# kawshik8/GAN-Image-Captioning

Measured on AMD Instinct MI355X. Metric: captions/sec (G+D train step), higher is better.
Workload: dtype bf16; 1 GPU; cfg2: adversarial G+D step, batch 64/GPU, 224x224 images, caption len 20, V=10000, E=H=512, 1-layer LSTM G, CNN-seq D (R=64,F=900), ResNet-50-shaped encoder, --conditional-gan 1; global_batch=64, caption_len=20, image_size=224, vocab=10000, conditional_gan=1, encoder=resnet50, step_impl=fused, parallelism=dp1

## Files before the change

### gan-image-captioning_amd/csrc/gemm.hip

```cpp
#include "gemm.h"
#include "conv3x3.h"
#include "conv1x1_stream.h"
#include "conv1x1_panel.h"
#include "conv1x1_pix.h"
#include "conv_stem.h"
#include "bn_fold.h"
#include "kernels.h"

#include <stdlib.h>

namespace gic {

namespace {

typedef __attribute__((address_space(3))) bf16x4 lds_bf16x4;
typedef unsigned int u32x4 __attribute__((ext_vector_type(4)));
typedef const __attribute__((address_space(1))) u32x4* gptr_u4;

__device__ __attribute__((aligned(16))) unsigned int g_zero16[4] = {0u, 0u, 0u, 0u};
typedef __attribute__((address_space(3))) void* lds_void_ptr;
typedef const __attribute__((address_space(1))) void* gbl_void_ptr;

#ifdef GIC_STAMPS
}
__device__ unsigned long long g_stamp[32];
namespace {
#define STAMP(i) do { if (tid == 0 && blockIdx.y == 0 && (blockIdx.x == 0 || blockIdx.x == gridDim.x - 1)) { \
  const int o_ = blockIdx.x == 0 ? 0 : 16; g_stamp[o_ + 2 * (i)] = __builtin_amdgcn_s_memtime(); g_stamp[o_ + 2 * (i) + 1] = __builtin_amdgcn_s_memrealtime(); } } while (0)
#define DBG d.dbg
#else
#define STAMP(i) do {} while (0)
#define DBG 0
#endif

template <typename T> struct GlobalPtr { typedef const __attribute__((address_space(1))) T* type; };

template <typename TI, typename TO, bool AKC, bool BKC, int BM, int BN, bool VEC, int EPI, bool CONV, bool PIPE>
__global__ __launch_bounds__(256) void gemm_kernel(const GemmDesc d, const int k_tiles_per_split) {
  static_assert(!CONV || (AKC && BKC && VEC), "the implicit-GEMM convolution loader is k-contiguous and vectorised");
  static_assert(!PIPE || (AKC && BKC && VEC), "the LDS-DMA pipeline needs k-contiguous 16-byte chunks");
  constexpr int SZ = sizeof(TI);
  constexpr int BK = 128 / SZ;
  constexpr int VE = 16 / SZ;
  constexpr int SA = PIPE ? 128 : (AKC ? 144 : BM * SZ + 16);
  constexpr int SB = PIPE ? 128 : (BKC ? 144 : BN * SZ + 16);
  constexpr int NSTAGE = PIPE ? 3 : 2;
  constexpr int A_BYTES = AKC ? BM * SA : BK * SA;
  constexpr int B_BYTES = BKC ? BN * SB : BK * SB;
  constexpr int BUF_BYTES = A_BYTES + B_BYTES;
  constexpr int TM = BM / 32, TN = BN / 32;
  constexpr int CA = BM / 32, CB = BN / 32;
  constexpr bool IS_BF16 = (SZ == 2);
  typedef typename GlobalPtr<TI>::type gptr_t;

  constexpr int EPI_BYTES = BM * (BN * (int)sizeof(TO) + 16) + 4 * (BN / 2) * 2 * 4;
  constexpr int SMEM_BYTES = NSTAGE * BUF_BYTES > EPI_BYTES ? NSTAGE * BUF_BYTES : EPI_BYTES;
  __shared__ __attribute__((aligned(16))) unsigned char smem[SMEM_BYTES];

  const int tid = threadIdx.x, lane = tid & 63, w = tid >> 6;
  STAMP(0);
  const int wr = w >> 1, wc = w & 1;
  const int lr = lane & 15, lg = lane >> 4;

  const int tiles_m = (d.M + BM - 1) / BM;
  const int nwg = gridDim.x;
  int bid = blockIdx.x;
  {
    const int q = nwg >> 3, r = nwg & 7, x = bid & 7;
    bid = (x < r ? x * (q + 1) : r * (q + 1) + (x - r) * q) + (bid >> 3);
  }
  const int bm0 = (bid % tiles_m) * BM;
  const int bn0 = (bid / tiles_m) * BN;

  gptr_t A = (gptr_t)d.A;
  gptr_t B = (gptr_t)d.B;
  const int M = d.M, N = d.N, K = d.K;
  const long lda = d.lda, ldb = d.ldb;

  f32x4 acc[TM][TN];
#pragma unroll
  for (int i = 0; i < TM; ++i)
#pragma unroll
    for (int j = 0; j < TN; ++j) acc[i][j] = (f32x4){0.f, 0.f, 0.f, 0.f};

  u32x4 ra[CA], rb[CB];

  long cv_base[CONV ? CA : 1];
  int cv_hi0[CONV ? CA : 1], cv_wi0[CONV ? CA : 1];
  int cv_r = 0, cv_s = 0, cv_c = 0;
  if constexpr (CONV) {
#pragma unroll
    for (int i = 0; i < CA; ++i) {
      const int m = bm0 + ((tid + i * 256) >> 3);
      const int mm = m < M ? m : 0;
      const int wo = mm % d.cWo, t = mm / d.cWo;
      const int ho = t % d.cHo, n = t / d.cHo;
      cv_hi0[i] = m < M ? ho * d.cStride - d.cPad : -(1 << 28);
      cv_wi0[i] = wo * d.cStride - d.cPad;
      cv_base[i] = ((long)n * d.cH + cv_hi0[i]) * d.cW + cv_wi0[i];
    }
    const int kchunk = PIPE ? ((tid & 7) ^ ((tid >> 4) & 7)) : (tid & 7);
    const int k = blockIdx.y * k_tiles_per_split * BK + kchunk * VE;
    cv_c = k % d.cCin;
    const int t = k / d.cCin;
    cv_s = t % d.cKW;
    cv_r = t / d.cKW;
  }

  auto gload = [&](int kt) {
    if constexpr (VEC) {
      const int k0 = kt * BK;
#pragma unroll
      for (int i = 0; i < CA; ++i) {
        const int c = tid + i * 256;
        ra[i] = (u32x4){0u, 0u, 0u, 0u};
        if constexpr (CONV) {
          const int hi = cv_hi0[i] + cv_r, wi = cv_wi0[i] + cv_s;
          if (cv_r < d.cKH && hi >= 0 && hi < d.cH && wi >= 0 && wi < d.cW)
            ra[i] = *(gptr_u4)(A + (cv_base[i] + (long)cv_r * d.cW + cv_s) * d.cCin + cv_c);
        } else if constexpr (AKC) {
          const int m = bm0 + (c >> 3), k = k0 + (c & 7) * VE;
          if (m < M && k < K) ra[i] = *(gptr_u4)(A + (long)m * lda + k);
        } else {
          constexpr int CPR = BM / VE;
          const int k = k0 + c / CPR, m = bm0 + (c % CPR) * VE;
          if (k < K && m < M) ra[i] = *(gptr_u4)(A + (long)k * lda + m);
        }
      }
#pragma unroll
      for (int i = 0; i < CB; ++i) {
        const int c = tid + i * 256;
        rb[i] = (u32x4){0u, 0u, 0u, 0u};
        if constexpr (BKC) {
          const int n = bn0 + (c >> 3), k = k0 + (c & 7) * VE;
          if (n < N && k < K) rb[i] = *(gptr_u4)(B + (long)n * ldb + k);
        } else {
          constexpr int CPR = BN / VE;
          const int k = k0 + c / CPR, n = bn0 + (c % CPR) * VE;
          if (k < K && n < N) rb[i] = *(gptr_u4)(B + (long)k * ldb + n);
        }
      }
      if constexpr (CONV) {
        cv_c += BK;
        while (cv_c >= d.cCin) {
          cv_c -= d.cCin;
          if (++cv_s == d.cKW) { cv_s = 0; ++cv_r; }
        }
      }
    }
  };

  auto sstore = [&](int kt, int buf) {
    unsigned char* sA = smem + buf * BUF_BYTES;
    unsigned char* sB = sA + A_BYTES;
    if constexpr (VEC) {
#pragma unroll
      for (int i = 0; i < CA; ++i) {
        const int c = tid + i * 256;
        if constexpr (AKC) {
          *(u32x4*)(sA + (c >> 3) * SA + (c & 7) * 16) = ra[i];
        } else {
          constexpr int CPR = BM / VE;
          *(u32x4*)(sA + (c / CPR) * SA + (c % CPR) * 16) = ra[i];
        }
      }
#pragma unroll
      for (int i = 0; i < CB; ++i) {
        const int c = tid + i * 256;
        if constexpr (BKC) {
          *(u32x4*)(sB + (c >> 3) * SB + (c & 7) * 16) = rb[i];
        } else {
          constexpr int CPR = BN / VE;
          *(u32x4*)(sB + (c / CPR) * SB + (c % CPR) * 16) = rb[i];
        }
      }
    } else {
      const int k0 = kt * BK;
      for (int e = tid; e < BM * BK; e += 256) {
        TI v = (TI)0.f;
        if constexpr (AKC) {
          const int row = e / BK, kk = e % BK;
          const int m = bm0 + row, k = k0 + kk;
          if (m < M && k < K) v = A[(long)m * lda + k];
          *(TI*)(sA + row * SA + kk * SZ) = v;
        } else {
          const int kk = e / BM, row = e % BM;
          const int m = bm0 + row, k = k0 + kk;
          if (m < M && k < K) v = A[(long)k * lda + m];
          *(TI*)(sA + kk * SA + row * SZ) = v;
        }
      }
      for (int e = tid; e < BN * BK; e += 256) {
        TI v = (TI)0.f;
        if constexpr (BKC) {
          const int row = e / BK, kk = e % BK;
          const int n = bn0 + row, k = k0 + kk;
          if (n < N && k < K) v = B[(long)n * ldb + k];
          *(TI*)(sB + row * SB + kk * SZ) = v;
        } else {
          const int kk = e / BN, row = e % BN;
          const int n = bn0 + row, k = k0 + kk;
          if (n < N && k < K) v = B[(long)k * ldb + n];
          *(TI*)(sB + kk * SB + row * SZ) = v;
        }
      }
    }
  };

  auto issue = [&](int kt, int buf) {
    if constexpr (PIPE) {
      unsigned char* sA = smem + buf * BUF_BYTES;
      unsigned char* sB = sA + A_BYTES;
      const int k0 = kt * BK;
      const int kc = ((tid & 7) ^ ((tid >> 4) & 7)) * VE;
      const int wbase = (tid & ~63) * 16;
#pragma unroll
      for (int i = 0; i < CA; ++i) {
        const int c = tid + i * 256;
        const TI* src = (const TI*)g_zero16;
        if constexpr (CONV) {
          const int hi = cv_hi0[i] + cv_r, wi = cv_wi0[i] + cv_s;
          if (cv_r < d.cKH && hi >= 0 && hi < d.cH && wi >= 0 && wi < d.cW)
            src = (const TI*)d.A + (cv_base[i] + (long)cv_r * d.cW + cv_s) * d.cCin + cv_c;
        } else {
          const int m = bm0 + (c >> 3), k = k0 + kc;
          if (m < M && k < K) src = (const TI*)d.A + (long)m * lda + k;
        }
        __builtin_amdgcn_global_load_lds((gbl_void_ptr)src, (lds_void_ptr)(sA + i * 4096 + wbase), 16, 0, 0);
      }
#pragma unroll
      for (int i = 0; i < CB; ++i) {
        const int c = tid + i * 256;
        const TI* src = (const TI*)g_zero16;
        const int n = bn0 + (c >> 3), k = k0 + kc;
        if (n < N && k < K) src = (const TI*)d.B + (long)n * ldb + k;
        __builtin_amdgcn_global_load_lds((gbl_void_ptr)src, (lds_void_ptr)(sB + i * 4096 + wbase), 16, 0, 0);
      }
      if constexpr (CONV) {
        cv_c += BK;
        while (cv_c >= d.cCin) {
          cv_c -= d.cCin;
          if (++cv_s == d.cKW) { cv_s = 0; ++cv_r; }
        }
      }
    }
  };

  auto compute = [&](int buf) {
    const unsigned char* sA = smem + buf * BUF_BYTES;
    const unsigned char* sB = sA + A_BYTES;
    if constexpr (IS_BF16) {
#pragma unroll
      for (int ks = 0; ks < BK / 32; ++ks) {
        bf16x8 fa[TM], fb[TN];
#pragma unroll
        for (int t = 0; t < TM; ++t) {
          const int r0 = wr * (BM / 2) + t * 16;
          if constexpr (PIPE) {
            fa[t] = *(const bf16x8*)(sA + (r0 + lr) * 128 + (((ks * 4 + lg) ^ (((r0 + lr) >> 1) & 7)) << 4));
          } else if constexpr (AKC) {
            fa[t] = *(const bf16x8*)(sA + (r0 + lr) * SA + ks * 64 + lg * 16);
          } else {
            const unsigned char* p0 = sA + (ks * 32 + lg * 8 + (lr >> 2)) * SA + (r0 + 4 * (lr & 3)) * 2;
            bf16x4 t0 = __builtin_amdgcn_ds_read_tr16_b64_v4bf16((lds_bf16x4*)p0);
            bf16x4 t1 = __builtin_amdgcn_ds_read_tr16_b64_v4bf16((lds_bf16x4*)(p0 + 4 * SA));
            fa[t] = __builtin_shufflevector(t0, t1, 0, 1, 2, 3, 4, 5, 6, 7);
          }
        }
#pragma unroll
        for (int t = 0; t < TN; ++t) {
          const int r0 = wc * (BN / 2) + t * 16;
          if constexpr (PIPE) {
            fb[t] = *(const bf16x8*)(sB + (r0 + lr) * 128 + (((ks * 4 + lg) ^ (((r0 + lr) >> 1) & 7)) << 4));
          } else if constexpr (BKC) {
            fb[t] = *(const bf16x8*)(sB + (r0 + lr) * SB + ks * 64 + lg * 16);
          } else {
            const unsigned char* p0 = sB + (ks * 32 + lg * 8 + (lr >> 2)) * SB + (r0 + 4 * (lr & 3)) * 2;
            bf16x4 t0 = __builtin_amdgcn_ds_read_tr16_b64_v4bf16((lds_bf16x4*)p0);
            bf16x4 t1 = __builtin_amdgcn_ds_read_tr16_b64_v4bf16((lds_bf16x4*)(p0 + 4 * SB));
            fb[t] = __builtin_shufflevector(t0, t1, 0, 1, 2, 3, 4, 5, 6, 7);
          }
        }
#pragma unroll
        for (int i = 0; i < TM; ++i)
#pragma unroll
          for (int j = 0; j < TN; ++j)
            acc[i][j] = __builtin_amdgcn_mfma_f32_16x16x32_bf16(fa[i], fb[j], acc[i][j], 0, 0, 0);
      }
    } else {
      float fa[TM][8], fb[TN][8];
#pragma unroll
      for (int t = 0; t < TM; ++t) {
        const int r0 = wr * (BM / 2) + t * 16;
        if constexpr (AKC) {
          const int sw = PIPE ? (((r0 + lr) >> 1) & 7) : 0;
          const float4 v0 = *(const float4*)(sA + (r0 + lr) * SA + (((2 * lg) ^ sw) << 4));
          const float4 v1 = *(const float4*)(sA + (r0 + lr) * SA + (((2 * lg + 1) ^ sw) << 4));
          fa[t][0] = v0.x; fa[t][1] = v0.y; fa[t][2] = v0.z; fa[t][3] = v0.w;
          fa[t][4] = v1.x; fa[t][5] = v1.y; fa[t][6] = v1.z; fa[t][7] = v1.w;
        } else {
#pragma unroll
          for (int s = 0; s < 8; ++s) fa[t][s] = *(const float*)(sA + (lg * 8 + s) * SA + (r0 + lr) * 4);
        }
      }
#pragma unroll
      for (int t = 0; t < TN; ++t) {
        const int r0 = wc * (BN / 2) + t * 16;
        if constexpr (BKC) {
          const int sw = PIPE ? (((r0 + lr) >> 1) & 7) : 0;
// ... 526 lines not shown
      __syncthreads();
      constexpr int CG = BN / 8;
      const int pc = tid % CG, pr = tid / CG;
      const int n0 = bn0 + pc * 8, m0 = bm0 + pr * 4;
      if (pr < BM / 4 && n0 < N && m0 < M) {
        float keep[4][8];
#pragma unroll
        for (int e = 0; e < 8; ++e) {
          keep[0][e] = keep[1][e] = keep[2][e] = keep[3][e] = 1.f;
          if (!d.mask && d.use_philox && n0 + e < N) {
            uint32_t r0, r1, r2, r3;
            Philox::gen4(d.seed_dev ? *d.seed_dev : d.seed, d.stream, (uint64_t)(m0 >> 2) * (uint64_t)N + (uint64_t)(n0 + e), r0, r1, r2, r3);
            keep[0][e] = Philox::u01(r0) >= d.drop_p ? 1.f : 0.f;
            keep[1][e] = Philox::u01(r1) >= d.drop_p ? 1.f : 0.f;
            keep[2][e] = Philox::u01(r2) >= d.drop_p ? 1.f : 0.f;
            keep[3][e] = Philox::u01(r3) >= d.drop_p ? 1.f : 0.f;
          }
        }
#pragma unroll
        for (int r = 0; r < 4; ++r) {
          const int m = m0 + r;
          if (m >= M) break;
          const float4 h0 = *(const float4*)(sH + (pr * 4 + r) * SH + pc * 8), h1 = *(const float4*)(sH + (pr * 4 + r) * SH + pc * 8 + 4);
          const float h[8] = {h0.x, h0.y, h0.z, h0.w, h1.x, h1.y, h1.z, h1.w};
          const bf16x8 xv = *(const bf16x8*)((const bf16_t*)d.X + (long)m * d.ldx + n0);
          bf16x8 yv;
          unsigned long long kb = 0ull;
#pragma unroll
          for (int e = 0; e < 8; ++e) {
            const bool live = n0 + e < N;
            const float sg = 1.f / (1.f + expf(-h[e]));
            const float y = sg * fmaxf(h[e], 0.f) + (1.f - sg) * (float)xv[e];
            float k = keep[r][e];
            if (d.mask && live) k = (float)d.mask[(long)m * d.ldmask + n0 + e];
            kb |= (unsigned long long)(live ? (unsigned)k : 0u) << (8 * e);
            yv[e] = (bf16_t)(live ? y * k * d.keep_scale : 0.f);
          }
          if (d.Hpre) {
            *(float4*)(d.Hpre + (long)m * d.ldh + n0) = h0;
            *(float4*)(d.Hpre + (long)m * d.ldh + n0 + 4) = h1;
          }
          if (d.mask_out) *(unsigned long long*)(d.mask_out + (long)m * d.ldmask_out + n0) = kb;
          *(bf16x8*)((bf16_t*)C + (long)m * d.ldc + n0) = yv;
        }
      }
      STAMP(5);
      return;
    }
#pragma unroll
    for (int i = 0; i < TM; ++i) {
#pragma unroll
      for (int j = 0; j < TN; ++j) {
        const int n = bn0 + wc * (BN / 2) + j * 16 + lr;
        if (n >= N) continue;
        const float bias = d.bias ? d.bias[n] : 0.f;
        const int mb = bm0 + wr * 32 + i * 16 + lg * 4;
        float keep4[4] = {1.f, 1.f, 1.f, 1.f};
        if (!d.mask && d.use_philox) {
          uint32_t r0, r1, r2, r3;
          Philox::gen4(d.seed_dev ? *d.seed_dev : d.seed, d.stream, (uint64_t)(mb >> 2) * (uint64_t)N + (uint64_t)n, r0, r1, r2, r3);
          keep4[0] = Philox::u01(r0) >= d.drop_p ? 1.f : 0.f;
          keep4[1] = Philox::u01(r1) >= d.drop_p ? 1.f : 0.f;
          keep4[2] = Philox::u01(r2) >= d.drop_p ? 1.f : 0.f;
          keep4[3] = Philox::u01(r3) >= d.drop_p ? 1.f : 0.f;
        }
#pragma unroll
        for (int r = 0; r < 4; ++r) {
          const int m = mb + r;
          if (m >= M) continue;
          const float v = d.alpha * acc[i][j][r] + bias;
          const float x = to_f32<bf16_t>(((const bf16_t*)d.X)[(long)m * d.ldx + n]);
          const float sg = 1.f / (1.f + expf(-v));
          const float y = sg * fmaxf(v, 0.f) + (1.f - sg) * x;
          if (d.Hpre) d.Hpre[(long)m * d.ldh + n] = v;
          float keep = keep4[r];
          if (d.mask) keep = (float)d.mask[(long)m * d.ldmask + n];
          if (d.mask_out) d.mask_out[(long)m * d.ldmask_out + n] = (uint8_t)keep;
          C[(long)m * d.ldc + n] = from_f32<TO>(y * keep * d.keep_scale);
        }
      }
    }
    STAMP(5);
    return;
  }
  unsigned char* sC = smem;
  float* sStat = (float*)(smem + BM * SC);
#pragma unroll
  for (int j = 0; j < TN; ++j) {
    const int nl = wc * (BN / 2) + j * 16 + lr;
    const int n = bn0 + nl;
    const float bias = (d.bias && n < N) ? d.bias[n] : 0.f;
    float st_s = 0.f, st_q = 0.f;
#pragma unroll
    for (int i = 0; i < TM; ++i) {
#pragma unroll
      for (int r = 0; r < 4; ++r) {
        const int ml = wr * 32 + i * 16 + lg * 4 + r;
        const float v = d.alpha * acc[i][j][r] + bias;
        *(TO*)(sC + ml * SC + nl * OSZ) = from_f32<TO>(v);
        if (EPI == EPI_BNSTATS && bm0 + ml < M) { st_s += v; st_q += v * v; }
      }
    }
    if constexpr (EPI == EPI_BNSTATS) {
      st_s += __shfl_xor(st_s, 16, 64); st_q += __shfl_xor(st_q, 16, 64);
      st_s += __shfl_xor(st_s, 32, 64); st_q += __shfl_xor(st_q, 32, 64);
      if (lg == 0) { sStat[(w * (BN / 2) + j * 16 + lr) * 2] = st_s; sStat[(w * (BN / 2) + j * 16 + lr) * 2 + 1] = st_q; }
    }
  }
  __syncthreads();
  STAMP(4);
  if constexpr (EPI == EPI_BNSTATS) {
    if (tid < BN) {
      const int cwc = tid / (BN / 2), cl = tid % (BN / 2), n = bn0 + tid;
      if (n < N) {
        float s0 = 0.f, q0 = 0.f;
#pragma unroll
        for (int r = 0; r < 4; ++r) {
          s0 += sStat[((r * 2 + cwc) * (BN / 2) + cl) * 2];
          q0 += sStat[((r * 2 + cwc) * (BN / 2) + cl) * 2 + 1];
        }
        float* stp = d.stats + (long)(blockIdx.x % d.stats_nrep) * 2 * N;
        atomicAdd(&stp[n], s0);
        atomicAdd(&stp[N + n], q0);
      }
    }
  }
  constexpr int CPR = BN / OVE;
  for (int c = tid; c < BM * CPR; c += NT) {
    const int ml = c / CPR, cc = c % CPR;
    const int m = bm0 + ml, n = bn0 + cc * OVE;
    if (m < M && n < N) {
      u32x4 v = *(const u32x4*)(sC + ml * SC + cc * 16);
      if (d.accumulate) {
        const u32x4 o = *(const u32x4*)(C + (long)m * d.ldc + n);
        TO* pv = (TO*)&v;
        const TO* po = (const TO*)&o;
#pragma unroll
        for (int e = 0; e < OVE; ++e) pv[e] = from_f32<TO>(to_f32<TO>(pv[e]) + to_f32<TO>(po[e]));
      }
      *(u32x4*)(C + (long)m * d.ldc + n) = v;
    }
  }
  STAMP(5);
}

template <typename TO, int EPI, bool CONV>
bool try_tile8(const GemmDesc& d_in, hipStream_t stream) {
  static const bool off = getenv("GIC_NO_TILE8") != nullptr;
  GemmDesc d = d_in;
  constexpr int OVE = 16 / (int)sizeof(TO);
  if (off || d.M < 128) return false;
  if (EPI != EPI_HIGHWAY && ((d.N % OVE) || (d.ldc % OVE) || (((uintptr_t)d.C) & 15))) return false;
  if (EPI == EPI_HIGHWAY && d.in_dtype != DT_BF16) return false;
  if (!CONV && ((long)cdiv(d.M, 128) * cdiv(d.N, 64) < 128 || d.K < 256)) return false;
  const long a_elems = CONV ? (long)(d.M / (d.cHo * d.cWo)) * d.cH * d.cW * d.cCin : (long)(d.M - 1) * d.lda + d.K;
  const long b_elems = (long)(d.N - 1) * d.ldb + d.K;
  if (a_elems * 2 >= (1l << 31) || b_elems * 2 >= (1l << 31)) return false;
  const long big_tiles = (long)cdiv(d.M, 128) * cdiv(d.N, 128);
  static const int big_min = [] { const char* e = getenv("GIC_TILE8_BIG_MIN"); return e ? atoi(e) : 160; }();
  static const int ns2_tiles = [] { const char* e = getenv("GIC_TILE8_NS2_TILES"); return e ? atoi(e) : 256; }();
  static const int min_nk = [] { const char* e = getenv("GIC_TILE8_MIN_NK"); return e ? atoi(e) : 1; }();
  if (cdiv(d.K, 64) < min_nk) return false;
  const unsigned ab = (unsigned)(a_elems * 2), bb = (unsigned)(b_elems * 2);
  d.n_fast = xcd_share_a(2 * (a_elems < (long)d.M * d.K ? a_elems : (long)d.M * d.K), 2l * d.N * d.K, cdiv(d.N, d.N >= 128 ? 128 : 64));
  if constexpr (EPI == EPI_BNSTATS && CONV) {
    if (d.in_stats && d.res) {
      if (d.cKH != 1 || d.cKW != 1 || d.cStride != 1 || d.cPad != 0 || d.cCin % 8 || d.cCin > 2048 || !d.in_gamma || !d.in_beta ||
          d.in_inv_count <= 0.f || (d.res_stats && (!d.res_gamma || !d.res_beta || d.res_inv_count <= 0.f)))
        return false;
      const bool n128 = d.N >= 128;
      const long tiles = n128 ? big_tiles : (long)cdiv(d.M, 128) * cdiv(d.N, 64);
      const dim3 grid((unsigned)tiles), block(512);
      static const int res_ns = [] { const char* e = getenv("GIC_TILE8_RES_NS"); return e ? atoi(e) : 1; }();
      if (d.cCin <= 512) {
        if (res_ns == 1) {
          if (n128) hipLaunchKernelGGL((tile8_kernel<TO, 128, EPI, CONV, 1, true, true, 512>), grid, block, 0, stream, d, ab, bb);
          else hipLaunchKernelGGL((tile8_kernel<TO, 64, EPI, CONV, 1, true, true, 512>), grid, block, 0, stream, d, ab, bb);
        } else {
          if (n128) hipLaunchKernelGGL((tile8_kernel<TO, 128, EPI, CONV, 2, true, true, 512>), grid, block, 0, stream, d, ab, bb);
          else hipLaunchKernelGGL((tile8_kernel<TO, 64, EPI, CONV, 2, true, true, 512>), grid, block, 0, stream, d, ab, bb);
        }
      } else {
        if (res_ns == 1) {
          if (n128) hipLaunchKernelGGL((tile8_kernel<TO, 128, EPI, CONV, 1, true, true, 2048>), grid, block, 0, stream, d, ab, bb);
          else hipLaunchKernelGGL((tile8_kernel<TO, 64, EPI, CONV, 1, true, true, 2048>), grid, block, 0, stream, d, ab, bb);
        } else {
          if (n128) hipLaunchKernelGGL((tile8_kernel<TO, 128, EPI, CONV, 2, true, true, 2048>), grid, block, 0, stream, d, ab, bb);
          else hipLaunchKernelGGL((tile8_kernel<TO, 64, EPI, CONV, 2, true, true, 2048>), grid, block, 0, stream, d, ab, bb);
        }
      }
      return true;
    }
    if (d.in_stats) {
      if (d.cCin % 8 || d.cCin > 1024 || !d.in_gamma || !d.in_beta || d.in_inv_count <= 0.f) return false;
      const int nk = cdiv(d.K, 64);
      const bool n128 = d.N >= 128 && big_tiles >= big_min;
      const long tiles = n128 ? big_tiles : (long)cdiv(d.M, 128) * cdiv(d.N, 64);
      const dim3 grid((unsigned)tiles), block(512);
      if (nk <= 4 && tiles > 512) {
        if (n128) hipLaunchKernelGGL((tile8_kernel<TO, 128, EPI, CONV, 1, true>), grid, block, 0, stream, d, ab, bb);
        else hipLaunchKernelGGL((tile8_kernel<TO, 64, EPI, CONV, 1, true>), grid, block, 0, stream, d, ab, bb);
      } else if (tiles > 256) {
        if (n128) hipLaunchKernelGGL((tile8_kernel<TO, 128, EPI, CONV, 2, true>), grid, block, 0, stream, d, ab, bb);
        else hipLaunchKernelGGL((tile8_kernel<TO, 64, EPI, CONV, 2, true>), grid, block, 0, stream, d, ab, bb);
      } else {
        if (n128) hipLaunchKernelGGL((tile8_kernel<TO, 128, EPI, CONV, 4, true>), grid, block, 0, stream, d, ab, bb);
        else hipLaunchKernelGGL((tile8_kernel<TO, 64, EPI, CONV, 4, true>), grid, block, 0, stream, d, ab, bb);
      }
      return true;
    }
  }
  static const int ns1_nk = [] { const char* e = getenv("GIC_TILE8_NS1_NK"); return e ? atoi(e) : 4; }();
  const int nk8 = cdiv(d.K, 64);
  if (EPI != EPI_HIGHWAY && nk8 <= ns1_nk && (d.N >= 128 ? big_tiles : (long)cdiv(d.M, 128) * cdiv(d.N, 64)) > 512) {
    if (d.N >= 128) hipLaunchKernelGGL((tile8_kernel<TO, 128, EPI, CONV, 1>), dim3((unsigned)big_tiles), dim3(512), 0, stream, d, ab, bb);
    else hipLaunchKernelGGL((tile8_kernel<TO, 64, EPI, CONV, 1>), dim3((unsigned)(cdiv(d.M, 128) * cdiv(d.N, 64))), dim3(512), 0, stream, d, ab, bb);
    return true;
  }
  if (d.N >= 128 && big_tiles >= big_min) {
    if (big_tiles > ns2_tiles) hipLaunchKernelGGL((tile8_kernel<TO, 128, EPI, CONV, 2>), dim3((unsigned)big_tiles), dim3(512), 0, stream, d, ab, bb);
    else hipLaunchKernelGGL((tile8_kernel<TO, 128, EPI, CONV, 4>), dim3((unsigned)big_tiles), dim3(512), 0, stream, d, ab, bb);
  } else {
    const long tiles = (long)cdiv(d.M, 128) * cdiv(d.N, 64);
    if (tiles > ns2_tiles) hipLaunchKernelGGL((tile8_kernel<TO, 64, EPI, CONV, 2>), dim3((unsigned)tiles), dim3(512), 0, stream, d, ab, bb);
    else hipLaunchKernelGGL((tile8_kernel<TO, 64, EPI, CONV, 4>), dim3((unsigned)tiles), dim3(512), 0, stream, d, ab, bb);
  }
  return true;
}


__global__ void zero2d_kernel(float* __restrict__ C, long ldc, int M, int N) {
  const long total = (long)M * N;
  for (long i = (long)blockIdx.x * blockDim.x + threadIdx.x; i < total; i += (long)gridDim.x * blockDim.x)
    C[(i / N) * ldc + (i % N)] = 0.f;
}

template <typename TI, typename TO, bool AKC, bool BKC, int BM, int BN, bool VEC, int EPI, bool CONV = false>
int launch(const GemmDesc& d, hipStream_t stream) {
  constexpr int BK = 128 / (int)sizeof(TI);
  const int tiles = cdiv(d.M, BM) * cdiv(d.N, BN);
  const int nk = cdiv(d.K, BK);
  int splits = 1;
  if (EPI == EPI_PLAIN && sizeof(TI) == 2 && sizeof(TO) == 4 && !d.no_split) {
    if (tiles < 24 && nk >= 8) {
      splits = 256 / tiles;
      if (splits > nk / 2) splits = nk / 2;
      if (splits > 16) splits = 16;
    } else if (tiles <= 192 && nk >= 32) {
      splits = 512 / tiles;
      if (splits > nk / 8) splits = nk / 8;
      if (splits > 16) splits = 16;
    } else if (!AKC && !BKC && tiles <= 192 && nk >= 16) {
      splits = 512 / tiles;
      if (splits > nk / 4) splits = nk / 4;
    } else if (tiles <= 320 && nk >= 64) {
      splits = 768 / tiles;
    }
    if (splits < 1) splits = 1;
    if (det_mode()) splits = (d.accumulate || splits < 2) ? 1 : 2;
  }
  int per = cdiv(nk, splits);
  splits = cdiv(nk, per);
  if (splits > 1 && !d.accumulate && !d.c_zeroed) {
    const long total = (long)d.M * d.N;
    const int g = (int)((total + 255) / 256 > 1024 ? 1024 : (total + 255) / 256);
    hipLaunchKernelGGL(zero2d_kernel, dim3(g), dim3(256), 0, stream, (float*)d.C, d.ldc, d.M, d.N);
  }
  constexpr bool CAN_PIPE = AKC && BKC && VEC;
  static const bool no_pipe = getenv("GIC_GEMM_NO_PIPE") != nullptr;
  const bool pipe = CAN_PIPE && per >= 6 && (long)tiles * splits <= 2 * 256 + 8 && !no_pipe;
  if constexpr (CAN_PIPE) {
    if (pipe) {
      hipLaunchKernelGGL((gemm_kernel<TI, TO, AKC, BKC, BM, BN, VEC, EPI, CONV, true>), dim3(tiles, splits), dim3(256), 0, stream, d, per);
      GIC_CHECK_LAUNCH("gemm");
      return GIC_OK;
    }
  }
  hipLaunchKernelGGL((gemm_kernel<TI, TO, AKC, BKC, BM, BN, VEC, EPI, CONV, false>), dim3(tiles, splits), dim3(256), 0, stream, d, per);
  GIC_CHECK_LAUNCH("gemm");
  return GIC_OK;
}

int big_tile_min() {
  static const int v = [] { const char* e = getenv("GIC_GEMM_BIG_MIN"); return e ? atoi(e) : 192; }();
  return v;
}

template <typename TI, typename TO, bool AKC, bool BKC, int EPI>
int pick_tile(const GemmDesc& d, bool vec, hipStream_t stream) {
  const long big_tiles = (long)cdiv(d.M, 128) * cdiv(d.N, 128);
  const bool big = big_tiles >= big_tile_min() && d.M >= 128 && d.N >= 128;
  if (big) {
    return vec ? launch<TI, TO, AKC, BKC, 128, 128, true, EPI>(d, stream)
               : launch<TI, TO, AKC, BKC, 128, 128, false, EPI>(d, stream);
  }
  return vec ? launch<TI, TO, AKC, BKC, 64, 64, true, EPI>(d, stream)
             : launch<TI, TO, AKC, BKC, 64, 64, false, EPI>(d, stream);
}

template <typename TI, typename TO, int EPI>
int pick_layout(const GemmDesc& d, bool vec, hipStream_t stream) {
  if constexpr (sizeof(TI) == 2) {
    if (d.a_kc && d.b_kc && vec && try_tile8<TO, EPI, false>(d, stream)) { GIC_CHECK_LAUNCH("gemm tile8"); return GIC_OK; }
  }
  if (d.a_kc && d.b_kc) return pick_tile<TI, TO, true, true, EPI>(d, vec, stream);
  if constexpr (EPI == EPI_PLAIN) {
    if (d.a_kc && !d.b_kc) return pick_tile<TI, TO, true, false, EPI>(d, vec, stream);
    if (!d.a_kc && !d.b_kc) return pick_tile<TI, TO, false, false, EPI>(d, vec, stream);
  }
  set_last_error("gemm: unsupported layout a_kc=%d b_kc=%d epi=%d", d.a_kc, d.b_kc, d.epi);
  return GIC_ERR_UNSUPPORTED;
}

template <typename TI, typename TO, int EPI>
int pick_conv(const GemmDesc& d, hipStream_t stream) {
  if constexpr (sizeof(TI) == 2 && sizeof(TO) == 2 && EPI == EPI_BNSTATS) {
    if (try_conv_stem(d, stream)) { GIC_CHECK_LAUNCH("conv stem"); return GIC_OK; }
    if (try_conv3x3_patch(d, stream)) { GIC_CHECK_LAUNCH("conv3x3 patch"); return GIC_OK; }
    if (try_conv1x1_stream(d, stream)) { GIC_CHECK_LAUNCH("conv1x1 stream"); return GIC_OK; }
    if (d.stats_only) return GIC_ERR_UNSUPPORTED;
    if (try_conv1x1_pix(d, stream)) { GIC_CHECK_LAUNCH("conv1x1 pix"); return GIC_OK; }
    if (try_conv1x1_panel(d, stream)) { GIC_CHECK_LAUNCH("conv1x1 panel"); return GIC_OK; }
    if (d.in_stats && d.cKH * d.cKW > 1) return GIC_ERR_UNSUPPORTED;
  }
  if constexpr (sizeof(TI) == 2) {
    if (try_tile8<TO, EPI, true>(d, stream)) { GIC_CHECK_LAUNCH("conv tile8"); return GIC_OK; }
  }
  if (d.in_stats) return GIC_ERR_UNSUPPORTED;
  const long big_tiles = (long)cdiv(d.M, 128) * cdiv(d.N, 128);
  if (big_tiles >= big_tile_min() && d.N >= 128) return launch<TI, TO, true, true, 128, 128, true, EPI, true>(d, stream);
  return launch<TI, TO, true, true, 64, 64, true, EPI, true>(d, stream);
}

template <typename TI, typename TO>
int pick_epi(const GemmDesc& d, bool vec, hipStream_t stream) {
  if (d.conv) {
    if (!vec || !d.a_kc || !d.b_kc) { set_last_error("gemm: convolution needs 16-B aligned NHWC / KRSC operands"); return GIC_ERR_UNSUPPORTED; }
    if constexpr (sizeof(TI) == sizeof(TO)) {
      if (d.epi == EPI_BNSTATS) return pick_conv<TI, TO, EPI_BNSTATS>(d, stream);
      if (d.epi == EPI_PLAIN) return pick_conv<TI, TO, EPI_PLAIN>(d, stream);
    }
    set_last_error("gemm: unsupported convolution epilogue / dtype");
    return GIC_ERR_UNSUPPORTED;
  }
  if (d.epi == EPI_PLAIN) return pick_layout<TI, TO, EPI_PLAIN>(d, vec, stream);
  if (d.epi == EPI_HIGHWAY) return pick_layout<TI, TO, EPI_HIGHWAY>(d, vec, stream);
  set_last_error("gemm: unknown epilogue %d", d.epi);
  return GIC_ERR_UNSUPPORTED;
}

bool aligned16(const void* p) { return (((uintptr_t)p) & 15) == 0; }

}

int gemm_gumbelmax(const GemmDesc& d0, hipStream_t stream) {
  GemmDesc d = d0;
  static const bool off = getenv("GIC_NO_TILE8") != nullptr || getenv("GIC_NO_FUSED_GUMBELMAX") != nullptr;
  GIC_CHECK_ARG(d.A && d.B && d.gm_rowkey && d.gm_bias, "gemm_gumbelmax: null operand");
  if (off || d.in_dtype != DT_BF16 || !d.a_kc || !d.b_kc || d.M < 128 || d.M % 4 || d.K % 8 || d.lda % 8 || d.ldb % 8 || !aligned16(d.A) ||
      !aligned16(d.B) || !aligned16(d.gm_bias) || (d.gm_u && (!aligned16(d.gm_u) || d.gm_ldu % 4)) || !(d.gm_temperature > 0.f))
    return GIC_ERR_UNSUPPORTED;
  const long a_elems = (long)(d.M - 1) * d.lda + d.K, b_elems = (long)(d.N - 1) * d.ldb + d.K;
  const long tiles = (long)cdiv(d.M, 128) * cdiv(d.N, 128);
  if (a_elems * 2 >= (1l << 31) || b_elems * 2 >= (1l << 31) || d.N < 128 || tiles < 160) return GIC_ERR_UNSUPPORTED;
  d.epi = EPI_GUMBELMAX;
  d.n_fast = xcd_share_a(2l * d.M * d.K, 2l * d.N * d.K, cdiv(d.N, 128));
  const unsigned ab = (unsigned)(a_elems * 2), bb = (unsigned)(b_elems * 2);
  if (tiles > 256) hipLaunchKernelGGL((tile8_kernel<float, 128, EPI_GUMBELMAX, false, 2>), dim3((unsigned)tiles), dim3(512), 0, stream, d, ab, bb);
  else hipLaunchKernelGGL((tile8_kernel<float, 128, EPI_GUMBELMAX, false, 4>), dim3((unsigned)tiles), dim3(512), 0, stream, d, ab, bb);
  GIC_CHECK_LAUNCH("gemm gumbelmax");
  return GIC_OK;
}

int gemm(const GemmDesc& d0, hipStream_t stream) {
  GemmDesc d = d0;
#ifdef GIC_STAMPS
  { const char* e = getenv("GIC_GEMM_DBG"); if (e) d.dbg = atoi(e); }
#endif
  GIC_CHECK_ARG(d.A && d.B && d.C, "gemm: null operand");
  GIC_CHECK_ARG(d.M >= 0 && d.N >= 0 && d.K >= 0, "gemm: negative dim");
  if (d.M == 0 || d.N == 0) return GIC_OK;
  {
    static const bool log = getenv("GIC_GEMM_LOG") != nullptr;
    if (log && !d.conv)
      fprintf(stderr, "[gemm] M=%d N=%d K=%d a_kc=%d b_kc=%d in=%d out=%d epi=%d acc=%d\n", d.M, d.N, d.K, d.a_kc, d.b_kc, d.in_dtype, d.out_dtype, d.epi,
              d.accumulate);
  }
  if (d.epi == EPI_HIGHWAY) GIC_CHECK_ARG(d.X, "gemm: highway epilogue needs X");
  const int sz = dtype_size(d.in_dtype);
  const int ve = 16 / sz;
  bool vec = aligned16(d.A) && aligned16(d.B) && (d.lda % ve == 0) && (d.ldb % ve == 0);
  if (d.conv) {
    const bool chunk_ok = (d.cCin % ve == 0) || (d.cPad == 0 && ve % d.cCin == 0 && (d.cKW * d.cCin) % ve == 0);
    GIC_CHECK_ARG(chunk_ok && d.K == d.cKH * d.cKW * d.cCin && d.K % ve == 0, "gemm: conv needs Cin %% %d == 0 (or a pre-padded NHWC4 stem) and K = KH*KW*Cin", ve);
    GIC_CHECK_ARG(d.epi != EPI_BNSTATS || d.stats, "gemm: EPI_BNSTATS needs a stats buffer");
    vec = aligned16(d.A) && aligned16(d.B) && (d.ldb % ve == 0);
  }
  if (d.a_kc || d.b_kc) vec = vec && (d.K % ve == 0);
  if (d.in_dtype == DT_F32 && d.out_dtype == DT_F32) return pick_epi<float, float>(d, vec, stream);
  if (d.in_dtype == DT_BF16 && d.out_dtype == DT_F32) return pick_epi<bf16_t, float>(d, vec, stream);
  if (d.in_dtype == DT_BF16 && d.out_dtype == DT_BF16) return pick_epi<bf16_t, bf16_t>(d, vec, stream);
  set_last_error("gemm: unsupported dtypes in=%d out=%d", d.in_dtype, d.out_dtype);
  return GIC_ERR_UNSUPPORTED;
}

}
#ifdef GIC_STAMPS
extern "C" int gic_debug_stamps(unsigned long long* out) {
  return (int)hipMemcpyFromSymbol(out, HIP_SYMBOL(gic::g_stamp), sizeof(unsigned long long) * 32);
}
#endif
```

Baseline: 26400 captions/s.

## Add split-K MFMA GEMM path for bf16 K-major operand layouts

Adds a new 128x128x64 bf16 GEMM kernel that handles non-K-contiguous operands by loading tiles straight into LDS with buffer loads and reading transposed fragments with ds_read_b64_tr_b16. It pipelines loads over 2 or 4 LDS stages and uses split-K with atomic fp32 accumulation when there are too few output tiles to fill the GPU. It is meant to speed up weight-gradient and transposed GEMMs that previously fell back to the generic tiled kernels. The costs are atomics, a separate zeroing launch and non-deterministic summation order, and it is gated by shape and alignment checks.

Result: faster. 26800 captions/s (median of 6 runs) (+1.5%).

```diff
diff --git a/gan-image-captioning_amd/csrc/gemm.hip b/gan-image-captioning_amd/csrc/gemm.hip
--- a/gan-image-captioning_amd/csrc/gemm.hip
+++ b/gan-image-captioning_amd/csrc/gemm.hip
@@ -5,6 +5,7 @@
 #include "conv1x1_pix.h"
 #include "conv_stem.h"
 #include "bn_fold.h"
+#include "gemm_kmajor.h"
 #include "kernels.h"
 
 #include <stdlib.h>
@@ -1137,6 +1138,7 @@
 int pick_layout(const GemmDesc& d, bool vec, hipStream_t stream) {
   if constexpr (sizeof(TI) == 2) {
     if (d.a_kc && d.b_kc && vec && try_tile8<TO, EPI, false>(d, stream)) { GIC_CHECK_LAUNCH("gemm tile8"); return GIC_OK; }
+    if (vec && try_kmajor8(d, stream)) { GIC_CHECK_LAUNCH("gemm kmajor8"); return GIC_OK; }
   }
   if (d.a_kc && d.b_kc) return pick_tile<TI, TO, true, true, EPI>(d, vec, stream);
   if constexpr (EPI == EPI_PLAIN) {
diff --git a/gan-image-captioning_amd/csrc/gemm_kmajor.h b/gan-image-captioning_amd/csrc/gemm_kmajor.h
--- /dev/null
+++ b/gan-image-captioning_amd/csrc/gemm_kmajor.h
@@ -0,0 +1,8 @@
+#pragma once
+#include "gemm.h"
+
+namespace gic {
+
+bool try_kmajor8(const GemmDesc& d, hipStream_t stream);
+
+}
diff --git a/gan-image-captioning_amd/csrc/gemm_kmajor.hip b/gan-image-captioning_amd/csrc/gemm_kmajor.hip
--- /dev/null
+++ b/gan-image-captioning_amd/csrc/gemm_kmajor.hip
@@ -0,0 +1,284 @@
+#include "gemm_kmajor.h"
+#include "kernels.h"
+
+#include <stdio.h>
+#include <stdlib.h>
+
+namespace gic {
+
+namespace {
+
+typedef __attribute__((address_space(3))) void* lds_void_ptr;
+typedef __attribute__((address_space(3))) unsigned char* lds_u8_ptr;
+typedef unsigned int u32x2 __attribute__((ext_vector_type(2)));
+typedef unsigned int u32x4 __attribute__((ext_vector_type(4)));
+
+__device__ __forceinline__ bf16x8 pack_frag(const u32x2 lo, const u32x2 hi) { return __builtin_bit_cast(bf16x8, ((u32x4){lo.x, lo.y, hi.x, hi.y})); }
+
+__device__ __forceinline__ int km_swz(const int k) { return ((k & 3) | ((k >> 1) & 4)) << 1; }
+
+template <bool AKC, bool BKC, int NS>
+__global__ __launch_bounds__(512) void kmajor8_kernel(const GemmDesc d, const unsigned a_bytes, const unsigned b_bytes, const int kt_per_split) {
+  constexpr int BM = 128, BN = 128, BK = 64, NT = 512;
+  constexpr int TM = 2, TN = 4;
+  constexpr int CH = BM * BK * 2 / 16 / NT;
+  constexpr int NL = 2 * CH;
+  constexpr int OP_BYTES = BM * BK * 2, STAGE = 2 * OP_BYTES;
+  constexpr int SC = BN * 4 + 16;
+  constexpr int EPI_BYTES = BM * SC;
+  constexpr int SMEM_BYTES = NS * STAGE > EPI_BYTES ? NS * STAGE : EPI_BYTES;
+  constexpr unsigned OOB = 0x80000000u;
+  static_assert(NS >= 2 && CH == 2 && SMEM_BYTES <= 160 * 1024, "kmajor8 LDS budget");
+  __shared__ __attribute__((aligned(16))) unsigned char smem[SMEM_BYTES];
+
+  const int tid = threadIdx.x, lane = tid & 63, w = tid >> 6;
+  const int wr = w >> 1, wc = w & 1;
+  const int lr = lane & 15, lg = lane >> 4;
+
+  const int tiles_m = (d.M + BM - 1) / BM, tiles_n = (d.N + BN - 1) / BN;
+  const int bid = xcd_run(blockIdx.x, gridDim.x);
+  const int bm0 = (d.n_fast ? bid / tiles_n : bid % tiles_m) * BM;
+  const int bn0 = (d.n_fast ? bid % tiles_n : bid / tiles_m) * BN;
+  const int M = d.M, N = d.N, K = d.K;
+  const unsigned lda = (unsigned)d.lda, ldb = (unsigned)d.ldb;
+  const int nk = (K + BK - 1) / BK;
+  const int kt0 = blockIdx.y * kt_per_split;
+  const int kt1 = min(nk, kt0 + kt_per_split);
+
+  const __amdgpu_buffer_rsrc_t rsA = __builtin_amdgcn_make_buffer_rsrc((void*)d.A, 0, (int)a_bytes, 0x00020000);
+  const __amdgpu_buffer_rsrc_t rsB = __builtin_amdgcn_make_buffer_rsrc((void*)d.B, 0, (int)b_bytes, 0x00020000);
+
+  const int a_kk = AKC ? ((tid & 7) ^ ((tid >> 4) & 7)) * 8 : (tid >> 4);
+  const int b_kk = BKC ? ((tid & 7) ^ ((tid >> 4) & 7)) * 8 : (tid >> 4);
+  unsigned a_off[CH], b_off[CH];
+  bool a_ok[CH], b_ok[CH];
+#pragma unroll
+  for (int i = 0; i < CH; ++i) {
+    if constexpr (AKC) {
+      const int m = bm0 + (tid >> 3) + i * 64;
+      a_ok[i] = m < M;
+      a_off[i] = (unsigned)m * lda + (unsigned)a_kk;
+    } else {
+      const int m = bm0 + ((tid & 15) ^ km_swz(tid >> 4)) * 8;
+      a_ok[i] = m < M;
+      a_off[i] = (unsigned)(a_kk + 32 * i) * lda + (unsigned)m;
+    }
+    if constexpr (BKC) {
+      const int n = bn0 + (tid >> 3) + i * 64;
+      b_ok[i] = n < N;
+      b_off[i] = (unsigned)n * ldb + (unsigned)b_kk;
+    } else {
+      const int n = bn0 + ((tid & 15) ^ km_swz(tid >> 4)) * 8;
+      b_ok[i] = n < N;
+      b_off[i] = (unsigned)(b_kk + 32 * i) * ldb + (unsigned)n;
+    }
+  }
+  const int wbase = (tid & ~63) * 16;
+
+  auto issue = [&](int kt, int st) {
+    unsigned char* sA = smem + st * STAGE;
+    unsigned char* sB = sA + OP_BYTES;
+    const bool live = kt < kt1;
+    const unsigned k0 = (unsigned)(kt * BK);
+#pragma unroll
+    for (int i = 0; i < CH; ++i) {
+      unsigned voff;
+      if constexpr (AKC) voff = (a_ok[i] & live & ((int)k0 + a_kk < K)) ? (a_off[i] + k0) * 2u : OOB;
+      else voff = (a_ok[i] & live & ((int)k0 + a_kk + 32 * i < K)) ? (a_off[i] + k0 * lda) * 2u : OOB;
+      __builtin_amdgcn_raw_ptr_buffer_load_lds(rsA, (lds_void_ptr)(sA + i * (NT * 16) + wbase), 16, (int)voff, 0, 0, 0);
+    }
+#pragma unroll
+    for (int i = 0; i < CH; ++i) {
+      unsigned voff;
+      if constexpr (BKC) voff = (b_ok[i] & live & ((int)k0 + b_kk < K)) ? (b_off[i] + k0) * 2u : OOB;
+      else voff = (b_ok[i] & live & ((int)k0 + b_kk + 32 * i < K)) ? (b_off[i] + k0 * ldb) * 2u : OOB;
+      __builtin_amdgcn_raw_ptr_buffer_load_lds(rsB, (lds_void_ptr)(sB + i * (NT * 16) + wbase), 16, (int)voff, 0, 0, 0);
+    }
+  };
+
+  auto frag_kc = [&](const unsigned char* s, const int r0, const int ks) -> bf16x8 {
+    const int row = r0 + lr;
+    return *(const bf16x8*)(s + row * 128 + (((ks * 4 + lg) ^ ((row >> 1) & 7)) << 4));
+  };
+  const unsigned sbase = (unsigned)(uintptr_t)(lds_u8_ptr)smem;
+  auto addr_km = [&](const int op, const int st, const int r0, const int ks) -> unsigned {
+    const int kr = ks * 32 + lg * 8 + (lr >> 2);
+    return sbase + (unsigned)(st * STAGE + op * OP_BYTES + kr * 256 + ((((r0 >> 3) + ((lr & 3) >> 1)) ^ km_swz(kr)) << 4) + ((lr & 1) << 3));
+  };
+
+  f32x4 acc[TM][TN];
+#pragma unroll
+  for (int i = 0; i < TM; ++i)
+#pragma unroll
+    for (int j = 0; j < TN; ++j) acc[i][j] = (f32x4){0.f, 0.f, 0.f, 0.f};
+
+  auto compute = [&](int st) {
+    const unsigned char* sA = smem + st * STAGE;
+    const unsigned char* sB = sA + OP_BYTES;
+#pragma unroll
+    for (int ks = 0; ks < 2; ++ks) {
+      bf16x8 fa[TM], fb[TN];
+      if constexpr (AKC) {
+#pragma unroll
+        for (int t = 0; t < TM; ++t) fa[t] = frag_kc(sA, wr * 32 + t * 16, ks);
+      }
+      if constexpr (BKC) {
+#pragma unroll
+        for (int t = 0; t < TN; ++t) fb[t] = frag_kc(sB, wc * 64 + t * 16, ks);
+      }
+      if constexpr (!AKC) {
+        u32x2 r[12];
+        asm volatile(
+            "ds_read_b64_tr_b16 %0, %12\n\tds_read_b64_tr_b16 %1, %12 offset:1024\n\t"
+            "ds_read_b64_tr_b16 %2, %13\n\tds_read_b64_tr_b16 %3, %13 offset:1024\n\t"
+            "ds_read_b64_tr_b16 %4, %14\n\tds_read_b64_tr_b16 %5, %14 offset:1024\n\t"
+            "ds_read_b64_tr_b16 %6, %15\n\tds_read_b64_tr_b16 %7, %15 offset:1024\n\t"
+            "ds_read_b64_tr_b16 %8, %16\n\tds_read_b64_tr_b16 %9, %16 offset:1024\n\t"
+            "ds_read_b64_tr_b16 %10, %17\n\tds_read_b64_tr_b16 %11, %17 offset:1024\n\t"
+            "s_waitcnt lgkmcnt(0)"
+            : "=&v"(r[0]), "=&v"(r[1]), "=&v"(r[2]), "=&v"(r[3]), "=&v"(r[4]), "=&v"(r[5]), "=&v"(r[6]), "=&v"(r[7]), "=&v"(r[8]),
+              "=&v"(r[9]), "=&v"(r[10]), "=&v"(r[11])
+            : "v"(addr_km(0, st, wr * 32, ks)), "v"(addr_km(0, st, wr * 32 + 16, ks)), "v"(addr_km(1, st, wc * 64, ks)),
+              "v"(addr_km(1, st, wc * 64 + 16, ks)), "v"(addr_km(1, st, wc * 64 + 32, ks)), "v"(addr_km(1, st, wc * 64 + 48, ks))
+            : "memory");
+#pragma unroll
+        for (int t = 0; t < TM; ++t) fa[t] = pack_frag(r[2 * t], r[2 * t + 1]);
+#pragma unroll
+        for (int t = 0; t < TN; ++t) fb[t] = pack_frag(r[4 + 2 * t], r[5 + 2 * t]);
+      } else if constexpr (!BKC) {
+        u32x2 r[8];
+        asm volatile(
+            "ds_read_b64_tr_b16 %0, %8\n\tds_read_b64_tr_b16 %1, %8 offset:1024\n\t"
+            "ds_read_b64_tr_b16 %2, %9\n\tds_read_b64_tr_b16 %3, %9 offset:1024\n\t"
+            "ds_read_b64_tr_b16 %4, %10\n\tds_read_b64_tr_b16 %5, %10 offset:1024\n\t"
+            "ds_read_b64_tr_b16 %6, %11\n\tds_read_b64_tr_b16 %7, %11 offset:1024\n\t"
+            "s_waitcnt lgkmcnt(0)"
+            : "=&v"(r[0]), "=&v"(r[1]), "=&v"(r[2]), "=&v"(r[3]), "=&v"(r[4]), "=&v"(r[5]), "=&v"(r[6]), "=&v"(r[7])
+            : "v"(addr_km(1, st, wc * 64, ks)), "v"(addr_km(1, st, wc * 64 + 16, ks)), "v"(addr_km(1, st, wc * 64 + 32, ks)),
+              "v"(addr_km(1, st, wc * 64 + 48, ks))
+            : "memory");
+#pragma unroll
+        for (int t = 0; t < TN; ++t) fb[t] = pack_frag(r[2 * t], r[2 * t + 1]);
+      }
+#pragma unroll
+      for (int i = 0; i < TM; ++i)
+#pragma unroll
+        for (int j = 0; j < TN; ++j) acc[i][j] = __builtin_amdgcn_mfma_f32_16x16x32_bf16(fa[i], fb[j], acc[i][j], 0, 0, 0);
+    }
+  };
+
+#pragma unroll
+  for (int s = 0; s < NS - 1; ++s) issue(kt0 + s, s);
+  int st = 0, st_fill = NS - 1;
+  for (int kt = kt0; kt < kt1; ++kt) {
+    asm volatile("s_waitcnt vmcnt(%0) lgkmcnt(0)" ::"n"((NS - 2) * NL) : "memory");
+    __builtin_amdgcn_s_barrier();
+    issue(kt + NS - 1, st_fill);
+    compute(st);
+    st = st == NS - 1 ? 0 : st + 1;
+    st_fill = st_fill == NS - 1 ? 0 : st_fill + 1;
+  }
+  asm volatile("s_waitcnt vmcnt(0)" ::: "memory");
+  __syncthreads();
+
+  float* __restrict__ C = (float*)d.C;
+  if (gridDim.y > 1) {
+#pragma unroll
+    for (int i = 0; i < TM; ++i)
+#pragma unroll
+      for (int j = 0; j < TN; ++j) {
+        const int n = bn0 + wc * 64 + j * 16 + lr;
+        const int mb = bm0 + wr * 32 + i * 16 + lg * 4;
+#pragma unroll
+        for (int r = 0; r < 4; ++r)
+          if (mb + r < M && n < N) atomicAdd(C + (long)(mb + r) * d.ldc + n, d.alpha * acc[i][j][r]);
+      }
+    return;
+  }
+  unsigned char* sC = smem;
+#pragma unroll
+  for (int i = 0; i < TM; ++i)
+#pragma unroll
+    for (int j = 0; j < TN; ++j) {
+      const int nl = wc * 64 + j * 16 + lr;
+#pragma unroll
+      for (int r = 0; r < 4; ++r) *(float*)(sC + (wr * 32 + i * 16 + lg * 4 + r) * SC + nl * 4) = d.alpha * acc[i][j][r];
+    }
+  __syncthreads();
+  constexpr int CPR = BN / 4;
+  for (int c = tid; c < BM * CPR; c += NT) {
+    const int ml = c / CPR, cc = c % CPR;
+    const int m = bm0 + ml, n = bn0 + cc * 4;
+    if (m < M && n < N) {
+      f32x4 v = *(const f32x4*)(sC + ml * SC + cc * 16);
+      f32x4* dst = (f32x4*)(C + (long)m * d.ldc + n);
+      if (d.accumulate) v += *dst;
+      *dst = v;
+    }
+  }
+}
+
+__global__ void kmajor8_zero_kernel(float* __restrict__ C, const long ldc, const int M, const int N4) {
+  for (int r = blockIdx.x; r < M; r += gridDim.x)
+    for (int c = threadIdx.x; c < N4; c += blockDim.x) *(f32x4*)(C + (long)r * ldc + 4 * c) = (f32x4){0.f, 0.f, 0.f, 0.f};
+}
+
+int env_int(const char* name, int dflt) {
+  const char* e = getenv(name);
+  return e ? atoi(e) : dflt;
+}
+
+}
+
+bool try_kmajor8(const GemmDesc& d_in, hipStream_t stream) {
+  static const bool off = getenv("GIC_NO_KMAJOR8") != nullptr;
+  static const bool log = getenv("GIC_GEMM_LOG") != nullptr;
+  static const int target = env_int("GIC_KMAJOR8_BLOCKS", 512);
+  static const int min_per = env_int("GIC_KMAJOR8_MIN_PER", 12);
+  GemmDesc d = d_in;
+  if (off || det_mode() || d.conv || d.epi != EPI_PLAIN || d.in_dtype != DT_BF16 || d.out_dtype != DT_F32 || d.bias || d.no_split) return false;
+  if (!d.a_kc && d.b_kc) return false;
+  if (d.a_kc && d.b_kc && d.K < 1024) return false;
+  const uintptr_t al = (uintptr_t)d.A | (uintptr_t)d.B | (uintptr_t)d.C;
+  if ((al & 15) || (d.lda % 8) || (d.ldb % 8) || (d.ldc % 4) || (d.N % 4) || ((d.a_kc || d.b_kc) && d.K % 8)) return false;
+  if (d.K < 256 || (double)d.M * d.N * d.K < (double)(1 << 26)) return false;
+  const long a_elems = d.a_kc ? (long)(d.M - 1) * d.lda + d.K : (long)(d.K - 1) * d.lda + ((d.M + 7) & ~7);
+  const long b_elems = d.b_kc ? (long)(d.N - 1) * d.ldb + d.K : (long)(d.K - 1) * d.ldb + ((d.N + 7) & ~7);
+  if (a_elems * 2 >= (1l << 31) || b_elems * 2 >= (1l << 31)) return false;
+  const int tiles_n = cdiv(d.N, 128);
+  const int tiles = cdiv(d.M, 128) * tiles_n;
+  const int nk = cdiv(d.K, 64);
+  int splits = 1;
+  if (tiles < target) {
+    splits = target / tiles;
+    if (splits > nk / min_per) splits = nk / min_per;
+    if (splits > 32) splits = 32;
+    if (splits < 1) splits = 1;
+  }
+  const int per = cdiv(nk, splits);
+  splits = cdiv(nk, per);
+  if ((long)tiles * splits < 256 || (double)cdiv(d.M, 128) * cdiv(d.N, 128) * 128 * 128 > 1.1 * d.M * d.N) return false;
+  if (splits > 1 && !d.accumulate && !d.c_zeroed) {
+    hipLaunchKernelGGL(kmajor8_zero_kernel, dim3((unsigned)(d.M < 4096 ? d.M : 4096)), dim3(128), 0, stream, (float*)d.C, d.ldc, d.M, d.N / 4);
+  }
+  d.n_fast = xcd_share_a(2l * d.M * d.K, 2l * d.N * d.K, tiles_n);
+  const unsigned ab = (unsigned)(a_elems * 2), bb = (unsigned)(b_elems * 2);
+  const dim3 grid((unsigned)tiles, (unsigned)splits), block(512);
+  const bool ns2 = (long)tiles * splits > 256;
+  if (d.a_kc && d.b_kc) {
+    if (ns2) hipLaunchKernelGGL((kmajor8_kernel<true, true, 2>), grid, block, 0, stream, d, ab, bb, per);
+    else hipLaunchKernelGGL((kmajor8_kernel<true, true, 4>), grid, block, 0, stream, d, ab, bb, per);
+  } else if (d.a_kc) {
+    if (ns2) hipLaunchKernelGGL((kmajor8_kernel<true, false, 2>), grid, block, 0, stream, d, ab, bb, per);
+    else hipLaunchKernelGGL((kmajor8_kernel<true, false, 4>), grid, block, 0, stream, d, ab, bb, per);
+  } else {
+    if (ns2) hipLaunchKernelGGL((kmajor8_kernel<false, false, 2>), grid, block, 0, stream, d, ab, bb, per);
+    else hipLaunchKernelGGL((kmajor8_kernel<false, false, 4>), grid, block, 0, stream, d, ab, bb, per);
+  }
+  if (log)
+    fprintf(stderr, "[gemm] route=kmajor8 M=%d N=%d K=%d a_kc=%d b_kc=%d tiles=%d splits=%d stages=%d\n", d.M, d.N, d.K, d.a_kc, d.b_kc, tiles, splits,
+            ns2 ? 2 : 4);
+  return true;
+}
+
+}
```
